# nevi-me/rust-dataframe

Hardware: AMD Instinct MI355X
Metric: rows/sec filter+sum over 1e9 f64 Arrow rows; %HBM bw at 1/2/4/8 GPU (higher is better)
Workload: dtype f64

## Files before the change

rust_dataframe_amd/csrc/rdf_capi.cpp:

```cpp
#include <hip/hip_runtime.h>

#include <algorithm>
#include <cmath>
#include <cstdarg>
#include <cstdio>
#include <chrono>
#include <functional>
#include <cstring>
#include <map>
#include <memory>
#include <mutex>
#include <condition_variable>
#include <string>
#include <thread>
#include <vector>
#include <sys/syscall.h>
#include <unistd.h>

#include "rdf_device.h"
#include "rdf_stage_copy.h"
#include "rdf_utf8.h"

using namespace rdfk;

// ... 3 lines not shown
struct Arena {
    char*  base = nullptr;
    size_t cap = 0, used = 0, wanted = 0;
    std::vector<void*> overflow;
};

struct Ctx {
    bool        ready = false;
    int         device = 0;
    hipStream_t own_stream = nullptr;
    hipStream_t stream = nullptr;
    hipStream_t copy_stream = nullptr;
    bool copy_pending = false;
    Arena       arena;
    char*       pinned = nullptr;
    size_t      pinned_cap = 0;
    std::string err;
    std::string last_kernel;
    bool   opt_spec = true;
    bool   opt_fast_filter = true;
    bool   opt_vec_bitmap = false;
    bool   opt_filter_one = true;
    int    opt_filter_gen = 2;
    int    opt_filter_block = 1;
    int    opt_interp_lean = 1;
    int    opt_filter_owned = 1;
    int    opt_filter_ends = 1;
    int    opt_filter_mixed = 0;
    int    opt_filter_short = 1;
    int    opt_filter_block_rows = 8192;
// ... 9 lines not shown
    int    opt_sort_msd = 1;
    int    opt_sort_sample = 1;
    int    opt_join_table = 2;
    int    opt_jit = 1;
    int    opt_take_rows = 1;
    int    opt_gb_skew_plan = 1;
    int    opt_gb_compact = 1;
    int64_t opt_comm_max_bytes = 0;
    int    opt_spec_blocks = 0;
    int    opt_spec_tile_rot = -1;
    int    opt_spec_xcd_swz = -1;
    int    opt_spec_grid_adj = 0;
    int    opt_gspec_blocks = 0;
    int    opt_gb_hot = 1;
    int    opt_gb_bucket = 0;
    int    opt_gb_partition = 3;
    bool   timing = false;
    std::vector<std::pair<hipEvent_t, hipEvent_t>> events;
    size_t events_used = 0;
    std::multimap<size_t, void*> pool_free;
    size_t pool_cached = 0;
    int64_t opt_stream_slab = 0;
    void*  sbuf_dev[2] = {nullptr, nullptr};
    void*  sbuf_pin[2] = {nullptr, nullptr};
    size_t sbuf_dev_cap = 0, sbuf_pin_cap = 0;
    hipEvent_t sbuf_ev[2] = {nullptr, nullptr};
    void*  dbuf_dev[2] = {nullptr, nullptr};
    void*  dbuf_pin[2] = {nullptr, nullptr};
    size_t dbuf_dev_cap = 0, dbuf_pin_cap = 0;
    hipEvent_t dbuf_ev[2] = {nullptr, nullptr};
// ... 5 lines not shown
    char* tab_pin = nullptr; size_t tab_pin_cap = 0, tab_pin_used = 0;
    bool   agg_comm_entered = false;
    ::rdf_comm* agg_comm = nullptr;
    ~Ctx();
};

thread_local Ctx g_ctx;

Ctx::~Ctx() {
    if (!ready || (long)syscall(SYS_gettid) == (long)getpid()) return;
    (void)hipSetDevice(device);
    if (stream) (void)hipStreamSynchronize(stream);
    for (void* p : arena.overflow) (void)hipFree(p);
    if (arena.base) (void)hipFree(arena.base);
    if (pinned) (void)hipHostFree(pinned);
    for (auto& kv : pool_free) (void)hipFree(kv.second);
    for (int b = 0; b < 2; ++b) { if (sbuf_dev[b]) (void)hipFree(sbuf_dev[b]); if (sbuf_pin[b]) (void)hipHostFree(sbuf_pin[b]); if (sbuf_ev[b]) (void)hipEventDestroy(sbuf_ev[b]); }
    if (tab_pin) (void)hipHostFree(tab_pin);
    if (d2h_stream) (void)hipStreamSynchronize(d2h_stream);
    for (int b = 0; b < 2; ++b) { if (dbuf_dev[b]) (void)hipFree(dbuf_dev[b]); if (dbuf_pin[b]) (void)hipHostFree(dbuf_pin[b]); if (dbuf_ev[b]) (void)hipEventDestroy(dbuf_ev[b]); }
    if (d2h_stream) (void)hipStreamDestroy(d2h_stream);
    for (auto& ev : events) { (void)hipEventDestroy(ev.first); (void)hipEventDestroy(ev.second); }
    if (copy_stream) { (void)hipStreamSynchronize(copy_stream); (void)hipStreamDestroy(copy_stream); }
    if (own_stream) (void)hipStreamDestroy(own_stream);
    ready = false;
}

rdf_status fail(rdf_status st, const char* fmt, ...) {
    char buf[512];
    va_list ap;
// ... 24 lines not shown
    if (e != hipSuccess || n <= 0)
        return fail(RDF_DEVICE_ERROR, "no HIP device visible (%s); librdf_mi355x has no CPU fallback",
                    e != hipSuccess ? hipGetErrorString(e) : "device count 0");
    HIP_TRY(hipGetDevice(&c.device));
    hipDeviceProp_t prop;
    HIP_TRY(hipGetDeviceProperties(&prop, c.device));
    if (strncmp(prop.gcnArchName, "gfx950", 6) != 0)
        return fail(RDF_DEVICE_ERROR, "device %d is %s; this library carries gfx950 (MI355X) code only", c.device, prop.gcnArchName);
    HIP_TRY(hipStreamCreateWithFlags(&c.own_stream, hipStreamNonBlocking));
    c.stream = c.own_stream;
    if (const char* e = getenv("RDF_SPEC_BLOCKS_PER_CU")) { const int v = atoi(e); if (v >= 0 && v <= 8) c.opt_spec_blocks = v; }
    if (const char* e = getenv("RDF_SPEC_TILE_ROT")) c.opt_spec_tile_rot = atoi(e);
    if (const char* e = getenv("RDF_SPEC_XCD_SWZ")) c.opt_spec_xcd_swz = atoi(e);
    if (const char* e = getenv("RDF_SPEC_GRID_ADJ")) c.opt_spec_grid_adj = atoi(e);
    if (const char* e = getenv("RDF_STREAM_TABLE_KERNEL")) c.opt_stream_table_kernel = atoi(e) != 0;
    if (const char* e = getenv("RDF_GSPEC_BLOCKS_PER_CU")) { const int v = atoi(e); if (v >= 0 && v <= 8) c.opt_gspec_blocks = v; }
    c.ready = true;
    return RDF_OK;
}

void arena_begin() {
    Arena& a = g_ctx.arena;
    for (void* p : a.overflow) (void)hipFree(p);
    a.overflow.clear();
    if (a.wanted > a.cap) {
        if (a.base) (void)hipFree(a.base);
        a.base = nullptr;
        a.cap = 0;
        size_t want = a.wanted + a.wanted / 4 + (1u << 20);
        void* p = nullptr;
// ... 11 lines not shown
        a.used += bytes;
        return RDF_OK;
    }
    void* p = nullptr;
    hipError_t e = hipMalloc(&p, bytes);
    if (e != hipSuccess) return fail(RDF_MEMORY_ERROR, "hipMalloc(%zu) failed: %s", bytes, hipGetErrorString(e));
    a.overflow.push_back(p);
    *out = p;
    return RDF_OK;
}
rdf_status pinned_reserve(size_t bytes) {
    Ctx& c = g_ctx;
    if (bytes <= c.pinned_cap) return RDF_OK;
    if (c.pinned && c.stream) (void)hipStreamSynchronize(c.stream);
    if (c.pinned) (void)hipHostFree(c.pinned);
    c.pinned = nullptr;
    c.pinned_cap = 0;
    size_t want = bytes + bytes / 2 + 4096;
    void* p = nullptr;
    hipError_t e = hipHostMalloc(&p, want, hipHostMallocDefault);
    if (e != hipSuccess) return fail(RDF_MEMORY_ERROR, "hipHostMalloc(%zu) failed: %s", want, hipGetErrorString(e));
    c.pinned = (char*)p;
    c.pinned_cap = want;
    return RDF_OK;
}

constexpr size_t kPoolGranule = (size_t)2 << 20;
constexpr size_t kPoolMaxCached = (size_t)96 << 30;
rdf_status pool_alloc(size_t bytes, void** out, size_t* got) {
    Ctx& c = g_ctx;
    const size_t gran = bytes < ((size_t)1 << 20) ? (size_t)4096 : kPoolGranule;
    const size_t want = (bytes + 256 + gran - 1) / gran * gran;
    auto it = c.pool_free.lower_bound(want);
    if (it != c.pool_free.end() && it->first <= want + want / 4 + gran) {
        *out = it->second; *got = it->first;
        c.pool_cached -= it->first;
        c.pool_free.erase(it);
        return RDF_OK;
// ... 749 lines not shown
                    if (op == RDF_OP_ADD) h = LH_I_ADD;
                    else if (op == RDF_OP_MUL) h = LH_I_MUL;
                    else if (op == RDF_OP_SUB) h = sw ? LH_I_RSUB : LH_I_SUB;
                }
            } break;
            default: break;
        }
        if (h == LH_NONE) return false;
        lean.code[i].swapped = (uint8_t)((in.swapped & 1) | (h << 1));
    }
    return true;
}

rdf_status launch_agg_pair(const EvalArgs* ea, const FilterAggF64Args* fa, int cmp, int feat, int grid, int nvalues,
                           const int* cls, AggPartial* partials, AggPartial* result, const char* spec_sig = nullptr,
                           const SpecArgs* sa = nullptr) {
    Ctx& c = g_ctx;
    KernelTimer kt;
    if (sa) {
        const bool jit = jit_find(spec_sig) != nullptr;
        c.last_kernel = std::string("spec_kernel<") + spec_sig + ">" + (jit ? " [compiled at run time]" : "");
        const hipError_t le = launch_spec(spec_sig, *sa, grid, c.stream);
        if (le != hipSuccess && jit) { (void)hipGetLastError(); return kRetryInterpreted; }
        if (le != hipSuccess) return fail(RDF_DEVICE_ERROR, "launch_spec: %s", hipGetErrorString(le));
    }
    else if (fa) { c.last_kernel = "filter_agg_f64_kernel"; HIP_TRY(launch_filter_agg_f64(*fa, cmp, grid, c.stream)); }
    else {
        EvalArgs lean;
        if (c.opt_interp_lean && feat == 0 && lean_assign(*ea, lean)) { c.last_kernel = "eval_kernel<AGG, lean>"; HIP_TRY(launch_eval_lean(lean, SINK_AGG, grid, c.stream, c.opt_interp_lean == 2)); }
        else { c.last_kernel = "eval_kernel<AGG>"; HIP_TRY(launch_eval(*ea, SINK_AGG, feat, grid, c.stream)); }
    }
    kt.stop();
    AggFinalArgs f;
    memset(&f, 0, sizeof f);
    f.partials = partials;
    f.result = result;
    f.nblocks = grid;
    f.nvalues = nvalues;
    for (int k = 0; k < nvalues; ++k) f.value_cls[k] = cls[k];
    HIP_TRY(launch_agg_final(f, c.stream));
    return RDF_OK;
}

void fill_agg_result(rdf_agg_result* r, int dt, const AggPartial& p) {
    memset(r, 0, sizeof *r);
    r->dtype = dt;
    r->count = p.cnt;
// ... 309 lines not shown
        tile_start.assign((size_t)nchunks + 1, 0);
        for (int64_t c = 0; c < nchunks; ++c) tile_start[(size_t)c + 1] = tile_start[(size_t)c] + (clen[(size_t)c] + kEvalTile - 1) / kEvalTile;
    }
    const int64_t ntiles = fc ? eval_tiles->ntiles : tile_start[(size_t)nchunks];
    int grid = (int)(ntiles < (int64_t)eval_grid_limit() ? ntiles : (int64_t)eval_grid_limit());

    const size_t n_nc = ps.sink == RDF_SINK_STORE ? (size_t)ps.nvalues * (size_t)nchunks : 0;
    const int gwords = grouped ? group_words(ps.ngroups, ps.nvalues) : 0;
    const size_t scratch_bytes = 16 + n_nc * 8 + ((size_t)grid + 4) * (grouped ? (size_t)gwords * 8 : (size_t)ps.nvalues * sizeof(AggPartial));
    void* scratch = nullptr;
    RDF_TRY(arena_alloc(scratch_bytes, &scratch));
    uint32_t* d_flags = (uint32_t*)scratch;
    int64_t* d_nullc = (int64_t*)((char*)scratch + 16);
    AggPartial* d_partials = (AggPartial*)((char*)scratch + 16 + n_nc * 8);
    AggPartial* d_result = d_partials + (size_t)grid * (size_t)ps.nvalues;
    HIP_TRY(hipMemsetAsync(scratch, 0, 16 + n_nc * 8, ctx.stream));

    EvalArgs ea;
    memset(&ea, 0, sizeof ea);
    ea.nchunks = nchunks;
    ea.ntiles = ntiles;
    ea.ncols = ncols;
    ea.nvalues = ps.nvalues;
    ea.ncode = (int)cc.code.size();
    ea.ntmp = cc.tmp_max;
    ea.flags = d_flags;
    ea.out_null_counts = d_nullc;
    ea.partials = d_partials;
    for (int k = 0; k < ncols; ++k) ea.col_dtype[k] = col_dtype[k];
    int cls[kMaxGroupValues] = {0, 0, 0, 0, 0, 0, 0, 0};
    for (int v = 0; v < ps.nvalues; ++v) { cls[v] = value_class(value_dtype[v]); ea.value_cls[v] = cls[v]; }
// ... 277 lines not shown
                    const DevChunkCol& y = in_dev[(size_t)vr.column];
                    const uintptr_t xa = (uintptr_t)((const double*)x.values + x.offset), ya = (uintptr_t)((const double*)y.values + y.offset);
                    if ((xa & 7) == 0 && (ya & 7) == 0 && (xa & 15) == (ya & 15)) {
                        memset(&fa, 0, sizeof fa);
                        fa.x = (const double*)x.values; fa.x_validity = x.validity; fa.x_offset = x.offset;
                        fa.y = (const double*)y.values; fa.y_validity = y.validity; fa.y_offset = y.offset;
                        fa.n = clen[0];
                        const uint64_t cu = cc.imm_for(*sc, RDF_F64);
                        memcpy(&fa.c, &cu, 8);
                        fa.partials = d_partials;
                        fast = true;
                    }
                }
            }
        }
        if (use_spec) {
            const rdf_status ls = launch_agg_pair(nullptr, nullptr, 0, 0, grid, ps.nvalues, cls, d_partials, d_result, sp.sig.c_str(), &sa);
            if (ls == kRetryInterpreted) return run_program(ps, cols, ncols, nchunks, outs, aggs, len_mismatch_msg, fc);
            RDF_TRY(ls);
        } else if (fast) {
            const int64_t per_block = (int64_t)kBlock * 4 * 2;
            int64_t want = (clen[0] + per_block - 1) / per_block;
            grid = (int)(want < (int64_t)eval_grid_limit() ? want : (int64_t)eval_grid_limit());
            if (grid < 1) grid = 1;
            d_result = d_partials + (size_t)grid * (size_t)ps.nvalues;
            RDF_TRY(launch_agg_pair(nullptr, &fa, cmp, 0, grid, 1, cls, d_partials, d_result));
        } else {
            RDF_TRY(launch_agg_pair(&ea, nullptr, 0, cc.feat(), grid, ps.nvalues, cls, d_partials, d_result));
        }
        if (ctx.agg_comm) {
            AggPartial hp[kMaxValues];
            uint32_t flags = 0;
            RDF_TRY(agg_dist_finish(*ctx.agg_comm, d_result, d_flags, ps.nvalues, cls, hp, &flags));
            if (flags & 2u) return fail(RDF_COMPUTE_ERROR, "pipeline_dist: another rank failed before the combine");
            if (flags & 1u) return fail(RDF_DIVIDE_BY_ZERO, "Divide by zero error");
            for (int v = 0; v < ps.nvalues; ++v) fill_agg_result(&aggs[v], value_dtype[v], hp[v]);
            return RDF_OK;
        }
        RDF_TRY(pinned_reserve(pin_off + 64 + sizeof(AggPartial) * kMaxValues));
        char* pin = ctx.pinned + pin_off;
        HIP_TRY(hipMemcpyAsync(pin, d_flags, 16, hipMemcpyDeviceToHost, ctx.stream));
        HIP_TRY(hipMemcpyAsync(pin + 64, d_result, sizeof(AggPartial) * (size_t)ps.nvalues, hipMemcpyDeviceToHost, ctx.stream));
        HIP_TRY(hipStreamSynchronize(ctx.stream));
        dbg.mark("kernel + result");
        uint32_t flags;
        memcpy(&flags, pin, 4);
        if (flags & 1u) return fail(RDF_DIVIDE_BY_ZERO, "Divide by zero error");
        for (int v = 0; v < ps.nvalues; ++v) {
            AggPartial p;
            memcpy(&p, pin + 64 + sizeof(AggPartial) * (size_t)v, sizeof p);
            fill_agg_result(&aggs[v], value_dtype[v], p);
        }
        return RDF_OK;
    }

    {
        KernelTimer kt;
// ... 125 lines not shown

rdf_status rdf_set_device(int32_t device) {
    Ctx& c = g_ctx;
    if (c.ready && c.device == device) return RDF_OK;
    if (c.ready) {
        (void)hipStreamSynchronize(c.stream);
        for (void* p : c.arena.overflow) (void)hipFree(p);
        c.arena.overflow.clear();
        if (c.arena.base) (void)hipFree(c.arena.base);
        c.arena = Arena();
        for (auto& ev : c.events) { (void)hipEventDestroy(ev.first); (void)hipEventDestroy(ev.second); }
        c.events.clear();
        c.events_used = 0;
        if (c.own_stream) (void)hipStreamDestroy(c.own_stream);
        c.own_stream = c.stream = nullptr;
        c.ready = false;
    }
    HIP_TRY(hipSetDevice(device));
    return ensure_ready();
}

rdf_status rdf_set_stream(void* hip_stream) {
    RDF_TRY(ensure_ready());
    g_ctx.stream = hip_stream ? (hipStream_t)hip_stream : g_ctx.own_stream;
    return RDF_OK;
}

rdf_status rdf_synchronize(void) {
    RDF_TRY(ensure_ready());
    HIP_TRY(hipStreamSynchronize(g_ctx.stream));
// ... 2414 lines not shown
    else if (strcmp(name, "gspec_blocks_per_cu") == 0) g_ctx.opt_gspec_blocks = (int)value;
    else if (strcmp(name, "filter_gen") == 0) g_ctx.opt_filter_gen = (int)value;
    else if (strcmp(name, "filter_fused") == 0) g_ctx.opt_filter_fused = (int)value;
    else if (strcmp(name, "filter_block") == 0) g_ctx.opt_filter_block = value == 3 ? 3 : value != 0;
    else if (strcmp(name, "interp_lean") == 0) g_ctx.opt_interp_lean = value == 2 ? 2 : value != 0;
    else if (strcmp(name, "sort_super") == 0) {
        if (value > 100) g_ctx.opt_sort_super_force = value > 164 ? 64 : (int)value - 100;
        else { g_ctx.opt_sort_super_force = 0; g_ctx.opt_sort_super = value < 1 ? 1 : value > 64 ? 64 : (int)value; }
    }
    else if (strcmp(name, "filter_owned") == 0) g_ctx.opt_filter_owned = value == 2 ? 2 : value != 0;
    else if (strcmp(name, "filter_ends") == 0) g_ctx.opt_filter_ends = value != 0;
    else if (strcmp(name, "filter_mixed") == 0) g_ctx.opt_filter_mixed = value == 2 ? 2 : value != 0;
    else if (strcmp(name, "filter_short") == 0) g_ctx.opt_filter_short = value != 0;
    else if (strcmp(name, "filter_block_rows") == 0) g_ctx.opt_filter_block_rows = value < 1 ? 1 : (int)value;
    else if (strcmp(name, "filter_lookback") == 0) g_ctx.opt_filter_lookback = value == 1 ? 1 : value == 2 ? 2 : 3;
    else if (strcmp(name, "comm_max_bytes") == 0) g_ctx.opt_comm_max_bytes = value;
    else if (strcmp(name, "stream_slab_bytes") == 0) g_ctx.opt_stream_slab = value;
    else return fail(RDF_INVALID_ARGUMENT, "unknown option %s", name);
    return RDF_OK;
}
int32_t rdf_spec_catalog_size(void) { return spec_catalog_size(); }
const char* rdf_jit_status(void) {
    thread_local std::string line;
    line = jit_status();
    return line.c_str();
}
const char* rdf_last_kernel(void) { return g_ctx.last_kernel.c_str(); }

rdf_status rdf_probe_stream(int32_t kind, const void* a, void* b, void* c, int64_t bytes, int32_t reps, double* best_gbps, char* shape, int32_t shape_len) {
    if (kind < 0 || kind > 2 || !a || (kind >= 1 && !b) || (kind == 2 && !c) || bytes < 16 || !best_gbps) return fail(RDF_INVALID_ARGUMENT, "probe_stream: kind 0..2 with its device buffers, bytes >= 16");
// ... 65 lines not shown
```

rust_dataframe_amd/csrc/rdf_common.hip.h:

```cpp
#pragma once
#include "rdf_device.h"

namespace rdfk {

__device__ __forceinline__ uint64_t uniform64(uint64_t v) {
    uint32_t lo = __builtin_amdgcn_readfirstlane((uint32_t)v);
    uint32_t hi = __builtin_amdgcn_readfirstlane((uint32_t)(v >> 32));
    return ((uint64_t)hi << 32) | lo;
}
__device__ __forceinline__ int wave_id() { return __builtin_amdgcn_readfirstlane((int)(threadIdx.x >> 6)); }

template <class T> using GlobalPtr = const T __attribute__((address_space(1)))*;
template <class T> using GlobalMutPtr = T __attribute__((address_space(1)))*;
template <class T> __device__ __forceinline__ GlobalPtr<T> as_global(const void* p) { return (GlobalPtr<T>)p; }
template <class T> using ConstPtr = const T __attribute__((address_space(4)))*;
template <class T> __device__ __forceinline__ ConstPtr<T> as_const(const void* p) { return (ConstPtr<T>)p; }
__device__ __forceinline__ DevChunkCol const_col(const DevChunkCol* table, int64_t i) {
    const ConstPtr<DevChunkCol> t = as_const<DevChunkCol>(table);
    DevChunkCol c;
    c.values = t[i].values; c.validity = t[i].validity; c.offset = t[i].offset;
    return c;
}
template <class T> __device__ __forceinline__ GlobalMutPtr<T> as_global_mut(void* p) { return (GlobalMutPtr<T>)p; }

// ... 116 lines not shown
    if (cls == CLS_F64) {
        sum = d2u(u2d(sum) + u2d(s2));
        mn = d2u(fmin(u2d(mn), u2d(mn2)));
        mx = d2u(fmax(u2d(mx), u2d(mx2)));
    } else if (cls == CLS_SIGNED) {
        sum += s2;
        mn = (uint64_t)((int64_t)mn2 < (int64_t)mn ? (int64_t)mn2 : (int64_t)mn);
        mx = (uint64_t)((int64_t)mx2 > (int64_t)mx ? (int64_t)mx2 : (int64_t)mx);
    } else {
        sum += s2;
        mn = mn2 < mn ? mn2 : mn;
        mx = mx2 > mx ? mx2 : mx;
    }
}

__device__ __forceinline__ void block_reduce_agg(int cls, uint64_t sum, uint64_t mn, uint64_t mx, int64_t cnt,
                                                 AggPartial* lds4, AggPartial* out) {
#pragma unroll
    for (int m = 32; m >= 1; m >>= 1) {
        uint64_t s2 = shfl_xor64(sum, m), mn2 = shfl_xor64(mn, m), mx2 = shfl_xor64(mx, m);
        int64_t c2 = (int64_t)shfl_xor64((uint64_t)cnt, m);
        agg_merge(cls, sum, mn, mx, cnt, s2, mn2, mx2, c2);
    }
    const int wave = threadIdx.x >> 6;
    __syncthreads();
    if ((threadIdx.x & 63) == 0) { lds4[wave].sum = sum; lds4[wave].mn = mn; lds4[wave].mx = mx; lds4[wave].cnt = cnt; }
    __syncthreads();
    if (threadIdx.x == 0) {
        uint64_t s = lds4[0].sum, a = lds4[0].mn, b = lds4[0].mx;
        int64_t c = lds4[0].cnt;
        for (int w = 1; w < kBlock / 64; ++w) agg_merge(cls, s, a, b, c, lds4[w].sum, lds4[w].mn, lds4[w].mx, lds4[w].cnt);
        out->sum = s; out->mn = a; out->mx = b; out->cnt = c;
    }
}

__device__ __forceinline__ void trig_reduce(double x, double& r, int& q) {
    const double kd = rint(x * 6.36619772367581382433e-01);
    q = (int)kd;
    double t = fma(-kd, 1.57079632673412561417e+00, x);
    t = fma(-kd, 6.07710050630396597660e-11, t);
    t = fma(-kd, 2.02226624871116645580e-21, t);
    r = fma(-kd, 8.47842766036889956997e-32, t);
}
__device__ __forceinline__ double trig_ksin(double r) {
    const double z = r * r, v = z * r;
    const double p = fma(z, fma(z, fma(z, fma(z, 1.58969099521155010221e-10, -2.50507602534068634195e-08), 2.75573137070700676789e-06),
                                -1.98412698298579493134e-04), 8.33333333332248946124e-03);
// ... 222 lines not shown
```

rust_dataframe_amd/csrc/rdf_device.h:

```cpp
#pragma once
#include "rdf_sort_map.h"
#include <stdint.h>
#include <hip/hip_runtime.h>

#include <string>
#include "../../include/rdf_mi355x.h"

namespace rdfk {

constexpr int kBlock = 256;
constexpr int kVPT = 4;
constexpr int kEvalTile = kBlock * kVPT;
constexpr int kFilterTile = 4096;
constexpr int kFilterTileSmall = 1024;
constexpr int kMaxCode = 56;
constexpr int kMaxCols = 8;
constexpr int kMaxFrameCols = 64;
constexpr int kPreCols = 4;
constexpr int kMaxTmp = 4;
constexpr int kMaxValues = RDF_MAX_VALUES;
constexpr int kMaxGroupValues = RDF_MAX_GROUP_VALUES;
constexpr int kMaxFilterCols = 8;

struct DevChunkCol {
// ... 19 lines not shown
    uint16_t src;
    uint64_t imm;
};
static_assert(sizeof(Instr) == 16, "Instr must stay 16 bytes");
enum : int {
    LH_NONE = 0, LH_LOAD, LH_STORE_TMP, LH_FILTER, LH_EMIT, LH_NOT, LH_CAST_I2F, LH_CAST_U2F,
    LH_F_GT, LH_F_GE, LH_F_EQ, LH_F_NE, LH_F_LT, LH_F_LE, LH_F_ADD, LH_F_SUB, LH_F_RSUB, LH_F_MUL, LH_F_DIV, LH_F_RDIV,
    LH_I_ADD, LH_I_SUB, LH_I_RSUB, LH_I_MUL, LH_AND, LH_OR
};

struct AggPartial {
    uint64_t sum, mn, mx;
    int64_t  cnt;
};
enum : int32_t { CLS_F64 = 0, CLS_SIGNED = 1, CLS_UNSIGNED = 2 };

enum : int32_t { SINK_STORE = 0, SINK_AGG = 1, SINK_GROUP = 2 };

struct EvalArgs {
    const DevChunkCol* cols;
    const int64_t*     chunk_tile_start;
    const int64_t*     chunk_len;
    DevOutChunk*       outs;
    int64_t*           out_null_counts;
    AggPartial*        partials;
    uint64_t*          group_partials;
    uint32_t*          flags;
    int64_t            nchunks, ntiles;
    DevChunkCol        inline_cols[kMaxCols];
    DevOutChunk        inline_outs[kMaxValues];
    int64_t            inline_len;
    int32_t            ncols, nvalues, ncode, ntmp;
    int32_t            col_dtype[kMaxCols];
    int32_t            value_cls[kMaxGroupValues];
    int32_t            ngroups, group_replicas;
    Instr              code[kMaxCode];
};

inline __host__ __device__ int group_words(int ngroups, int nvalues) { return (ngroups + 1) * (2 * nvalues + 1); }

constexpr int kGSpecCols = 8;
constexpr int kGSpecImm = 8;
struct GSpecArgs {
    const DevChunkCol* cols_tab;
    const int64_t*     chunk_tile_start;
    const int64_t*     chunk_len;
    DevChunkCol        cols[kGSpecCols];
    int32_t            col_map[kGSpecCols];
    int64_t            nchunks, ntiles, n;
    uint64_t           imm[kGSpecImm];
// ... 11 lines not shown
};

struct AggFinalArgs {
    const AggPartial* partials;
    AggPartial*       result;
    int32_t           nblocks, nvalues;
    int32_t           value_cls[kMaxValues];
};

struct FilterAggF64Args {
    const double*  x;   const uint8_t* x_validity;   int64_t x_offset;
    const double*  y;   const uint8_t* y_validity;   int64_t y_offset;
    int64_t        n;
    double         c;
    AggPartial*    partials;
};

constexpr int kSpecCols = 8;
constexpr int kSpecImm = 8;
struct SpecArgs {
    DevChunkCol        cols[kSpecCols];
    DevOutChunk        out;
    const DevChunkCol* cols_tab;
    const DevOutChunk* outs_tab;
    const int64_t*     chunk_tile_start;
    const int64_t*     chunk_len;
    int64_t            nchunks, ntiles;
    int64_t            n;
    uint64_t           tile_inv;
    uint64_t           imm[kSpecImm];
    int64_t*           out_null_count;
    AggPartial*        partials;
    uint32_t*          flags;
    int32_t            vec_bitmap;
    int32_t            rt[8];
    int32_t            alias[kSpecCols];
    int64_t            tile_rot;
    int32_t            xcd_swz, pad0;
};

struct MaskTables {
    const DevChunkCol* mask;
    const int64_t*     chunk_tile_start;
    const int64_t*     chunk_len;
    int64_t            nchunks, ntiles;
};
struct FilterArgs {
    MaskTables         t;
    const DevChunkCol* cols;
    DevOutChunk*       outs;
    int64_t*           out_null_counts;
    const int64_t*     tile_scan;
    int32_t            ncols;
// ... 545 lines not shown
```

rust_dataframe_amd/csrc/rdf_eval.hip:

```cpp
#include "rdf_common.hip.h"

#ifndef RDF_FEAT
#error "compile with -DRDF_FEAT=0|1|2"
#endif

namespace rdfk {


__device__ __forceinline__ uint64_t cast_value(int from, int to, uint64_t x, bool& ok) {
    ok = true;
    if (from == to) return x;
    double f = 0.0;
    bool src_float = false;
    if (from == RDF_F64) { f = u2d(x); src_float = true; }
    else if (from == RDF_F32) { f = (double)u2f(x); src_float = true; }
    if (to == RDF_BOOL) return src_float ? (uint64_t)(f != 0.0) : (uint64_t)(x != 0);
    if (to == RDF_F64) {
        if (src_float) return d2u(f);
        return d2u(dt_is_signed(from) ? (double)(int64_t)x : (double)x);
    }
    if (to == RDF_F32) {
        if (from == RDF_F64) return f2u((float)u2d(x));
        return f2u(dt_is_signed(from) ? (float)(int64_t)x : (float)x);
    }
// ... 666 lines not shown
            const bool fsum = w < a.nvalues * gS && a.value_cls[(w / gS) & (kMaxGroupValues - 1)] == CLS_F64;
            uint64_t acc0 = gtab[w];
            for (int r = 1; r < a.group_replicas; ++r) {
                const uint64_t x = gtab[(size_t)r * gwords + w];
                acc0 = fsum ? d2u(u2d(acc0) + u2d(x)) : acc0 + x;
            }
            a.group_partials[(size_t)blockIdx.x * gwords + w] = acc0;
        }
    }
    if (SINK == SINK_AGG) {
#pragma unroll
        for (int k = 0; k < NVAL; ++k)
            if (k < a.nvalues)
                block_reduce_agg(a.value_cls[k], g_sum[k], g_mn[k], g_mx[k], g_cnt[k], red_lds,
                                 &a.partials[(int64_t)blockIdx.x * a.nvalues + k]);
    }
}


template <int SINK, int NPRE, int NVAL>
static void launch_one(const EvalArgs& a, int grid, size_t lds, hipStream_t s) {
    hipLaunchKernelGGL((eval_kernel<RDF_FEAT, SINK, NPRE, NVAL>), dim3(grid), dim3(kBlock), lds, s, a);
}
template <int SINK>
static void launch_shape(const EvalArgs& a, int npre, int nval, int grid, size_t lds, hipStream_t s) {
    if (nval <= 1) {
        if (npre <= 1) launch_one<SINK, 1, 1>(a, grid, lds, s);
        else if (npre <= 2) launch_one<SINK, 2, 1>(a, grid, lds, s);
        else launch_one<SINK, 4, 1>(a, grid, lds, s);
    } else if (nval <= 2) {
// ... 22 lines not shown
```

rust_dataframe_amd/csrc/rdf_eval_lean.hip:

```cpp
#include "rdf_common.hip.h"

namespace rdfk {

#define RDF_ROWS _Pragma("unroll") for (int j = 0; j < kVPT; ++j)

typedef uint64_t lean_u64x2 __attribute__((ext_vector_type(2)));
typedef uint32_t lean_u32x2 __attribute__((ext_vector_type(2)));

__device__ __forceinline__ uint32_t lean_nibble(const uint64_t (&w)[kVPT], int lane) {
    const uint32_t q = (uint32_t)lane >> 4, sh = ((uint32_t)lane & 15u) * 4u;
    const uint32_t c0 = (uint32_t)(w[0] >> sh), c1 = (uint32_t)(w[1] >> sh), c2 = (uint32_t)(w[2] >> sh), c3 = (uint32_t)(w[3] >> sh);
    const uint32_t m0 = 0u - (uint32_t)(q == 0), m1 = 0u - (uint32_t)(q == 1), m2 = 0u - (uint32_t)(q == 2), m3 = 0u - (uint32_t)(q == 3);
    return ((c0 & m0) | (c1 & m1) | (c2 & m2) | (c3 & m3)) & 15u;
}

__device__ __forceinline__ void lean_load8(const DevChunkCol cc, int64_t rw, int64_t clen, bool full, uint64_t (&v)[kVPT], uint32_t& valid) {
    const int lane = threadIdx.x & 63;
    const GlobalPtr<uint64_t> base = as_global<uint64_t>(cc.values) + cc.offset;
    if (full && (((uintptr_t)cc.values + (uintptr_t)(cc.offset + rw) * 8) & 15) == 0) {
        const GlobalPtr<lean_u64x2> p = (GlobalPtr<lean_u64x2>)(base + rw + (int64_t)lane * kVPT);
        const lean_u64x2 a0 = __builtin_nontemporal_load(p), a1 = __builtin_nontemporal_load(p + 1);
        v[0] = a0[0]; v[1] = a0[1]; v[2] = a1[0]; v[3] = a1[1];
    } else {
        const int64_t last = clen - 1;
// ... 54 lines not shown
__device__ __forceinline__ void lean_block_reduce(int cls, uint64_t sum, uint64_t mn, uint64_t mx, int64_t cnt, AggPartial* lds4, AggPartial* out) {
#pragma unroll
    for (int m = 32; m >= 1; m >>= 1) {
        const uint64_t s2 = shfl_xor64(sum, m), mn2 = shfl_xor64(mn, m), mx2 = shfl_xor64(mx, m);
        const int64_t c2 = (int64_t)shfl_xor64((uint64_t)cnt, m);
        agg_merge(cls, sum, mn, mx, cnt, s2, mn2, mx2, c2);
    }
    sum = uniform64(sum); mn = uniform64(mn); mx = uniform64(mx); cnt = (int64_t)uniform64((uint64_t)cnt);
    const int wave = wave_id();
    __syncthreads();
    lds4[wave].sum = sum; lds4[wave].mn = mn; lds4[wave].mx = mx; lds4[wave].cnt = cnt;
    __syncthreads();
    uint64_t s = lds4[0].sum, lo = lds4[0].mn, hi = lds4[0].mx;
    int64_t c = lds4[0].cnt;
    for (int w = 1; w < kBlock / 64; ++w) agg_merge(cls, s, lo, hi, c, lds4[w].sum, lds4[w].mn, lds4[w].mx, lds4[w].cnt);
    out->sum = s; out->mn = lo; out->mx = hi; out->cnt = c;
}

__device__ __forceinline__ void lean_store_words(uint8_t* bitmap, int64_t rw, int64_t rows_left, uint32_t nibble, int lane) {
    uint64_t x = (uint64_t)(nibble & 15u) << (((uint32_t)lane & 15u) * 4u);
#pragma unroll
    for (int m = 1; m < 16; m <<= 1) x |= shfl_xor64(x, m);
    const int64_t span = rows_left < 0 ? 0 : rows_left < (int64_t)kVPT * 64 ? rows_left : (int64_t)kVPT * 64;
    const int nwords = (int)((span + 63) >> 6);
    const __amdgpu_buffer_rsrc_t rs = __builtin_amdgcn_make_buffer_rsrc(bitmap + (rw >> 6) * 8, 0, nwords * 8, 0x00020000);
    lean_u32x2 w;
    w[0] = (uint32_t)x; w[1] = (uint32_t)(x >> 32);
    const uint32_t off = ((uint32_t)lane & 15u) == 0 ? ((uint32_t)lane >> 4) * 8u : 0x7FFFFFF0u;
    __builtin_amdgcn_raw_buffer_store_b64(w, rs, (int)off, 0, 0);
}

// ... 238 lines not shown
                        } else {
                            const uint64_t* tv = tmp_vals + (size_t)src * R * kBlock + tid;
                            RDF_ROWS_R opnd[r] = tv[r * kBlock];
                            opv = tmp_valid[src * kBlock + tid];
                        }
                        accv &= opv;
                        lean_bin<R>(h, acc, [&](int r) { return opnd[r]; }, accv & inr, err);
                    }
                } break;
            }
        }
        tile = ntile;
        have = nhave;
    }

    if (__ballot(err != 0) != 0) *(volatile uint32_t*)a.flags = 1u;
    if constexpr (SINK == SINK_AGG) {
#pragma unroll
        for (int k = 0; k < NVAL; ++k)
            if (k < a.nvalues)
                lean_block_reduce(a.value_cls[k], g_sum[k], g_mn[k], g_mx[k], g_cnt[k], red_lds, &a.partials[(int64_t)blockIdx.x * a.nvalues + k]);
    }
}

template <int SINK, int NPRE, int NVAL, int T>
static void lean_launch_one(const EvalArgs& a, int grid, hipStream_t s) {
    const size_t lds = (size_t)a.ntmp * ((size_t)T * kVPT * kBlock * 8 + kBlock * 4);
    hipLaunchKernelGGL((eval_lean_kernel<SINK, NPRE, NVAL, T>), dim3(grid), dim3(kBlock), lds, s, a);
}

hipError_t launch_eval_lean(const EvalArgs& a, int sink, int grid, hipStream_t s, bool one_tile) {
    const int npre = a.ncols, nval = a.nvalues;
    const bool two = !one_tile && (npre <= 1 || (npre <= 2 && sink == SINK_AGG)) && (size_t)a.ntmp * (2 * kVPT * kBlock * 8 + kBlock * 4) <= 65536;
    if (sink == SINK_STORE) {
        if (npre <= 1) { if (two) lean_launch_one<SINK_STORE, 1, 1, 2>(a, grid, s); else lean_launch_one<SINK_STORE, 1, 1, 1>(a, grid, s); }
        else if (npre <= 2) lean_launch_one<SINK_STORE, 2, 1, 1>(a, grid, s);
// ... 14 lines not shown
```

rust_dataframe_amd/csrc/rdf_kernels.hip:

```cpp
#include "rdf_common.hip.h"
#include "rdf_join_place.h"

namespace rdfk {

__global__ __launch_bounds__(kBlock) void agg_final_kernel(const AggFinalArgs a) {
    __shared__ AggPartial red_lds[kBlock / 64];
    for (int k = 0; k < a.nvalues; ++k) {
        const int cls = a.value_cls[k];
        uint64_t s, mn, mx;
        int64_t cnt;
        agg_init(cls, s, mn, mx, cnt);
        for (int b = threadIdx.x; b < a.nblocks; b += kBlock) {
            const AggPartial p = a.partials[(int64_t)b * a.nvalues + k];
            agg_merge(cls, s, mn, mx, cnt, p.sum, p.mn, p.mx, p.cnt);
        }
        block_reduce_agg(cls, s, mn, mx, cnt, red_lds, &a.result[k]);
        __syncthreads();
    }
}


template <int CMP>
__device__ __forceinline__ bool cmp_f64(double x, double c) {
    if (CMP == RDF_OP_GT) return x > c;
    if (CMP == RDF_OP_GE) return x >= c;
    if (CMP == RDF_OP_EQ) return x == c;
    if (CMP == RDF_OP_NE) return x != c;
    if (CMP == RDF_OP_LT) return x < c;
    return x <= c;
}

struct F64Agg {
    double sum, mn, mx;
// ... 58 lines not shown
#pragma unroll
        for (int u = 0; u < kFU; ++u) {
            const int64_t i = wbase + u * 64 + lane;
            uint32_t bits = i < nvec ? 3u : 0u;
            if (HASV) {
                const int sh = (2 * lane) & 63;
                if (a.x_validity) bits &= (uint32_t)((lane < 32 ? wx[2 * u] : wx[2 * u + 1]) >> sh) & 3u;
                if (!SAME && a.y_validity) bits &= (uint32_t)((lane < 32 ? wy[2 * u] : wy[2 * u + 1]) >> sh) & 3u;
            }
            const dvec2 yy = SAME ? vx[u] : vy[u];
            if ((bits & 1u) && cmp_f64<CMP>(vx[u].x, a.c)) g.add(yy.x);
            if ((bits & 2u) && cmp_f64<CMP>(vx[u].y, a.c)) g.add(yy.y);
        }
    }
    block_reduce_agg(CLS_F64, d2u(g.sum), d2u(g.mn), d2u(g.mx), g.cnt, red_lds, &a.partials[blockIdx.x]);
}

template <int WW> constexpr int filter_tile_rows() { return WW * 64 * (kBlock / 64); }
static_assert(filter_tile_rows<16>() == kFilterTile && filter_tile_rows<4>() == kFilterTileSmall, "tile sizes of the two instantiations");

template <int WW>
__device__ __forceinline__ void locate_tile(const MaskTables& t, int64_t tile, int64_t& c, int64_t& r0, int64_t& clen) {
    c = t.nchunks == 1 ? 0 : find_chunk_tile(t.chunk_tile_start, t.nchunks, tile);
    r0 = (tile - t.chunk_tile_start[c]) * filter_tile_rows<WW>();
    clen = t.chunk_len[c];
}

template <int kWW>
__device__ __forceinline__ void keep_words(const DevChunkCol& m, int64_t rw, int64_t clen, uint64_t (&kw)[kWW]) {
    load_windows<kWW>((const uint8_t*)m.values, m.offset + rw, clen - rw, kw);
// ... 1760 lines not shown
```

rust_dataframe_amd/csrc/rdf_spec_kernel.hip.h:

```cpp
#pragma once
#include <map>
#include <string>
#include <type_traits>

#include "rdf_expr.hip.h"

namespace rdfk {


template <int DT> struct AggT;
template <> struct AggT<RDF_F64> {
    double sum, mn, mx; int64_t cnt;
    static constexpr int cls = CLS_F64;
    __device__ __forceinline__ void init() { sum = 0.0; mn = mx = __longlong_as_double(0x7FF8000000000000ll); cnt = 0; }
    __device__ __forceinline__ void add(double v) { sum += v; mn = fmin(mn, v); mx = fmax(mx, v); ++cnt; }
    __device__ __forceinline__ uint64_t s() const { return d2u(sum); }
    __device__ __forceinline__ uint64_t a() const { return d2u(mn); }
    __device__ __forceinline__ uint64_t b() const { return d2u(mx); }
};
template <> struct AggT<RDF_I64> {
    uint64_t sum; int64_t mn, mx; int64_t cnt;
    static constexpr int cls = CLS_SIGNED;
    __device__ __forceinline__ void init() { sum = 0; mn = INT64_MAX; mx = INT64_MIN; cnt = 0; }
    __device__ __forceinline__ void add(int64_t v) { sum += (uint64_t)v; mn = v < mn ? v : mn; mx = v > mx ? v : mx; ++cnt; }
// ... 405 lines not shown
                }
#pragma unroll
                for (int e = 0; e < RV; ++e) nulls += (uint32_t)__popcll(inb[e] & ~vb[e]);
            }
            if (lane < R && rw + 64 * lane < n) {
                if constexpr (V0::dt == RDF_BOOL) as_global_mut<uint64_t>(out.values)[(rw >> 6) + lane] = word_val;
                if (out.validity) as_global_mut<uint64_t>(out.validity)[(rw >> 6) + lane] = word_vld;
            }
        }
    }
    if (c.err) atomicOr(a.flags, c.err);
    if constexpr (P::SINK == SINK_AGG) {
        constexpr int nv = has_v1 ? 2 : 1;
        block_reduce_agg(g0.cls, g0.s(), g0.a(), g0.b(), g0.cnt, red_lds, &a.partials[(int64_t)blockIdx.x * nv]);
        if constexpr (has_v1) block_reduce_agg(g1.cls, g1.s(), g1.a(), g1.b(), g1.cnt, red_lds, &a.partials[(int64_t)blockIdx.x * nv + 1]);
    } else {
        if (cur_chunk >= 0 && lane == 0 && nulls) atomicAdd((unsigned long long*)&a.out_null_count[cur_chunk], (unsigned long long)nulls);
    }
}


typedef void (*SpecLaunch)(const SpecArgs&, int, hipStream_t);
struct SpecEntry { SpecLaunch launch; int rows_per_tile; };
std::map<std::string, SpecEntry>& spec_registry();

template <class P>
static void launch_prog(const SpecArgs& a, int grid, hipStream_t s) {
    hipLaunchKernelGGL((spec_kernel<P>), dim3(grid), dim3(kBlock), 0, s, a);
}
template <class P>
// ... 119 lines not shown
```

Baseline: 841.6 billion.

## Fold final aggregate into main kernel via last-block ticket and host-mapped output

Measured after the change: 841.8 billion, median of 6. Within noise of the previous version (+0.0%).

```diff
diff --git a/rust_dataframe_amd/csrc/rdf_capi.cpp b/rust_dataframe_amd/csrc/rdf_capi.cpp
--- a/rust_dataframe_amd/csrc/rdf_capi.cpp
+++ b/rust_dataframe_amd/csrc/rdf_capi.cpp
@@ -41,6 +41,7 @@
     bool copy_pending = false;
     Arena       arena;
     char*       pinned = nullptr;
+    char*       pinned_dev = nullptr;
     size_t      pinned_cap = 0;
     std::string err;
     std::string last_kernel;
@@ -80,6 +81,9 @@
     int    opt_gspec_blocks = 0;
     int    opt_gb_hot = 1;
     int    opt_gb_bucket = 0;
+    int    opt_agg_fold = 1;
+    void*  fold_state = nullptr;
+    uint64_t fold_t0 = 0;
     int    opt_gb_partition = 3;
     bool   timing = false;
     std::vector<std::pair<hipEvent_t, hipEvent_t>> events;
@@ -115,6 +119,7 @@
     for (void* p : arena.overflow) (void)hipFree(p);
     if (arena.base) (void)hipFree(arena.base);
     if (pinned) (void)hipHostFree(pinned);
+    if (fold_state) (void)hipFree(fold_state);
     for (auto& kv : pool_free) (void)hipFree(kv.second);
     for (int b = 0; b < 2; ++b) { if (sbuf_dev[b]) (void)hipFree(sbuf_dev[b]); if (sbuf_pin[b]) (void)hipHostFree(sbuf_pin[b]); if (sbuf_ev[b]) (void)hipEventDestroy(sbuf_ev[b]); }
     if (tab_pin) (void)hipHostFree(tab_pin);
@@ -169,6 +174,7 @@
     if (const char* e = getenv("RDF_SPEC_XCD_SWZ")) c.opt_spec_xcd_swz = atoi(e);
     if (const char* e = getenv("RDF_SPEC_GRID_ADJ")) c.opt_spec_grid_adj = atoi(e);
     if (const char* e = getenv("RDF_STREAM_TABLE_KERNEL")) c.opt_stream_table_kernel = atoi(e) != 0;
+    if (const char* e = getenv("RDF_AGG_FOLD")) c.opt_agg_fold = atoi(e) != 0;
     if (const char* e = getenv("RDF_GSPEC_BLOCKS_PER_CU")) { const int v = atoi(e); if (v >= 0 && v <= 8) c.opt_gspec_blocks = v; }
     c.ready = true;
     return RDF_OK;
@@ -210,14 +216,35 @@
     if (bytes <= c.pinned_cap) return RDF_OK;
     if (c.pinned && c.stream) (void)hipStreamSynchronize(c.stream);
     if (c.pinned) (void)hipHostFree(c.pinned);
-    c.pinned = nullptr;
+    c.pinned = c.pinned_dev = nullptr;
     c.pinned_cap = 0;
     size_t want = bytes + bytes / 2 + 4096;
     void* p = nullptr;
     hipError_t e = hipHostMalloc(&p, want, hipHostMallocDefault);
     if (e != hipSuccess) return fail(RDF_MEMORY_ERROR, "hipHostMalloc(%zu) failed: %s", want, hipGetErrorString(e));
+    void* pd = nullptr;
+    e = hipHostGetDevicePointer(&pd, p, 0);
+    if (e != hipSuccess) { (void)hipHostFree(p); return fail(RDF_MEMORY_ERROR, "hipHostGetDevicePointer: %s", hipGetErrorString(e)); }
     c.pinned = (char*)p;
+    c.pinned_dev = (char*)pd;
     c.pinned_cap = want;
+    return RDF_OK;
+}
+
+rdf_status agg_fold_state(AggFold* fold) {
+    Ctx& c = g_ctx;
+    if (!c.fold_state) {
+        void* p = nullptr;
+        HIP_TRY(hipMalloc(&p, 256));
+        const hipError_t e = hipMemsetAsync(p, 0, 256, c.stream) == hipSuccess ? hipStreamSynchronize(c.stream) : hipGetLastError();
+        if (e != hipSuccess) { (void)hipFree(p); return fail(RDF_DEVICE_ERROR, "agg_fold state: %s", hipGetErrorString(e)); }
+        c.fold_state = p;
+        c.fold_t0 = 0;
+    }
+    memset(fold, 0, sizeof *fold);
+    fold->ticket = (unsigned long long*)c.fold_state;
+    fold->flags = (uint32_t*)((char*)c.fold_state + 64);
+    fold->t0 = c.fold_t0;
     return RDF_OK;
 }
 
@@ -997,23 +1024,36 @@
 
 rdf_status launch_agg_pair(const EvalArgs* ea, const FilterAggF64Args* fa, int cmp, int feat, int grid, int nvalues,
                            const int* cls, AggPartial* partials, AggPartial* result, const char* spec_sig = nullptr,
-                           const SpecArgs* sa = nullptr) {
+                           const SpecArgs* sa = nullptr, const AggFold* fold = nullptr) {
     Ctx& c = g_ctx;
     KernelTimer kt;
     if (sa) {
         const bool jit = jit_find(spec_sig) != nullptr;
         c.last_kernel = std::string("spec_kernel<") + spec_sig + ">" + (jit ? " [compiled at run time]" : "");
-        const hipError_t le = launch_spec(spec_sig, *sa, grid, c.stream);
+        SpecArgs a = *sa;
+        if (fold) a.fold = *fold;
+        const hipError_t le = launch_spec(spec_sig, a, grid, c.stream);
         if (le != hipSuccess && jit) { (void)hipGetLastError(); return kRetryInterpreted; }
         if (le != hipSuccess) return fail(RDF_DEVICE_ERROR, "launch_spec: %s", hipGetErrorString(le));
     }
-    else if (fa) { c.last_kernel = "filter_agg_f64_kernel"; HIP_TRY(launch_filter_agg_f64(*fa, cmp, grid, c.stream)); }
+    else if (fa) {
+        c.last_kernel = "filter_agg_f64_kernel";
+        FilterAggF64Args a = *fa;
+        if (fold) a.fold = *fold;
+        HIP_TRY(launch_filter_agg_f64(a, cmp, grid, c.stream));
+    }
     else {
         EvalArgs lean;
-        if (c.opt_interp_lean && feat == 0 && lean_assign(*ea, lean)) { c.last_kernel = "eval_kernel<AGG, lean>"; HIP_TRY(launch_eval_lean(lean, SINK_AGG, grid, c.stream, c.opt_interp_lean == 2)); }
-        else { c.last_kernel = "eval_kernel<AGG>"; HIP_TRY(launch_eval(*ea, SINK_AGG, feat, grid, c.stream)); }
+        EvalArgs a = *ea;
+        if (fold) a.fold = *fold;
+        if (c.opt_interp_lean && feat == 0 && lean_assign(a, lean)) { c.last_kernel = "eval_kernel<AGG, lean>"; HIP_TRY(launch_eval_lean(lean, SINK_AGG, grid, c.stream, c.opt_interp_lean == 2)); }
+        else { c.last_kernel = "eval_kernel<AGG>"; HIP_TRY(launch_eval(a, SINK_AGG, feat, grid, c.stream)); }
     }
     kt.stop();
+    if (fold) {
+        c.fold_t0 += (uint64_t)grid;
+        return RDF_OK;
+    }
     AggFinalArgs f;
     memset(&f, 0, sizeof f);
     f.partials = partials;
@@ -1353,7 +1393,8 @@
     int64_t* d_nullc = (int64_t*)((char*)scratch + 16);
     AggPartial* d_partials = (AggPartial*)((char*)scratch + 16 + n_nc * 8);
     AggPartial* d_result = d_partials + (size_t)grid * (size_t)ps.nvalues;
-    HIP_TRY(hipMemsetAsync(scratch, 0, 16 + n_nc * 8, ctx.stream));
+    const bool agg_fold = ps.sink == RDF_SINK_AGG && !grouped && ctx.opt_agg_fold;
+    if (!agg_fold) HIP_TRY(hipMemsetAsync(scratch, 0, 16 + n_nc * 8, ctx.stream));
 
     EvalArgs ea;
     memset(&ea, 0, sizeof ea);
@@ -1661,8 +1702,20 @@
                 }
             }
         }
+        AggFold fold;
+        if (agg_fold) {
+            RDF_TRY(pinned_reserve(pin_off + 64 + sizeof(AggPartial) * kMaxValues));
+            RDF_TRY(agg_fold_state(&fold));
+            fold.result = d_result;
+            fold.call_flags = d_flags;
+            fold.host = ctx.pinned_dev + pin_off;
+            fold.nvalues = ps.nvalues;
+            for (int v = 0; v < ps.nvalues; ++v) fold.value_cls[v] = cls[v];
+            ea.flags = sa.flags = fold.flags;
+        }
+        const AggFold* fp = agg_fold ? &fold : nullptr;
         if (use_spec) {
-            const rdf_status ls = launch_agg_pair(nullptr, nullptr, 0, 0, grid, ps.nvalues, cls, d_partials, d_result, sp.sig.c_str(), &sa);
+            const rdf_status ls = launch_agg_pair(nullptr, nullptr, 0, 0, grid, ps.nvalues, cls, d_partials, d_result, sp.sig.c_str(), &sa, fp);
             if (ls == kRetryInterpreted) return run_program(ps, cols, ncols, nchunks, outs, aggs, len_mismatch_msg, fc);
             RDF_TRY(ls);
         } else if (fast) {
@@ -1671,9 +1724,10 @@
             grid = (int)(want < (int64_t)eval_grid_limit() ? want : (int64_t)eval_grid_limit());
             if (grid < 1) grid = 1;
             d_result = d_partials + (size_t)grid * (size_t)ps.nvalues;
-            RDF_TRY(launch_agg_pair(nullptr, &fa, cmp, 0, grid, 1, cls, d_partials, d_result));
+            if (agg_fold) fold.result = d_result;
+            RDF_TRY(launch_agg_pair(nullptr, &fa, cmp, 0, grid, 1, cls, d_partials, d_result, nullptr, nullptr, fp));
         } else {
-            RDF_TRY(launch_agg_pair(&ea, nullptr, 0, cc.feat(), grid, ps.nvalues, cls, d_partials, d_result));
+            RDF_TRY(launch_agg_pair(&ea, nullptr, 0, cc.feat(), grid, ps.nvalues, cls, d_partials, d_result, nullptr, nullptr, fp));
         }
         if (ctx.agg_comm) {
             AggPartial hp[kMaxValues];
@@ -1686,8 +1740,10 @@
         }
         RDF_TRY(pinned_reserve(pin_off + 64 + sizeof(AggPartial) * kMaxValues));
         char* pin = ctx.pinned + pin_off;
-        HIP_TRY(hipMemcpyAsync(pin, d_flags, 16, hipMemcpyDeviceToHost, ctx.stream));
-        HIP_TRY(hipMemcpyAsync(pin + 64, d_result, sizeof(AggPartial) * (size_t)ps.nvalues, hipMemcpyDeviceToHost, ctx.stream));
+        if (!agg_fold) {
+            HIP_TRY(hipMemcpyAsync(pin, d_flags, 16, hipMemcpyDeviceToHost, ctx.stream));
+            HIP_TRY(hipMemcpyAsync(pin + 64, d_result, sizeof(AggPartial) * (size_t)ps.nvalues, hipMemcpyDeviceToHost, ctx.stream));
+        }
         HIP_TRY(hipStreamSynchronize(ctx.stream));
         dbg.mark("kernel + result");
         uint32_t flags;
@@ -1843,6 +1899,9 @@
         c.events_used = 0;
         if (c.own_stream) (void)hipStreamDestroy(c.own_stream);
         c.own_stream = c.stream = nullptr;
+        if (c.fold_state) (void)hipFree(c.fold_state);
+        c.fold_state = nullptr;
+        c.fold_t0 = 0;
         c.ready = false;
     }
     HIP_TRY(hipSetDevice(device));
@@ -4287,6 +4346,7 @@
     else if (strcmp(name, "filter_short") == 0) g_ctx.opt_filter_short = value != 0;
     else if (strcmp(name, "filter_block_rows") == 0) g_ctx.opt_filter_block_rows = value < 1 ? 1 : (int)value;
     else if (strcmp(name, "filter_lookback") == 0) g_ctx.opt_filter_lookback = value == 1 ? 1 : value == 2 ? 2 : 3;
+    else if (strcmp(name, "agg_fold") == 0) g_ctx.opt_agg_fold = value != 0;
     else if (strcmp(name, "comm_max_bytes") == 0) g_ctx.opt_comm_max_bytes = value;
     else if (strcmp(name, "stream_slab_bytes") == 0) g_ctx.opt_stream_slab = value;
     else return fail(RDF_INVALID_ARGUMENT, "unknown option %s", name);
diff --git a/rust_dataframe_amd/csrc/rdf_common.hip.h b/rust_dataframe_amd/csrc/rdf_common.hip.h
--- a/rust_dataframe_amd/csrc/rdf_common.hip.h
+++ b/rust_dataframe_amd/csrc/rdf_common.hip.h
@@ -154,6 +154,13 @@
     }
 }
 
+__device__ __forceinline__ void agg_store_partial(AggPartial* out, uint64_t s, uint64_t mn, uint64_t mx, int64_t c) {
+    __hip_atomic_store(&out->sum, s, __ATOMIC_RELAXED, __HIP_MEMORY_SCOPE_AGENT);
+    __hip_atomic_store(&out->mn, mn, __ATOMIC_RELAXED, __HIP_MEMORY_SCOPE_AGENT);
+    __hip_atomic_store(&out->mx, mx, __ATOMIC_RELAXED, __HIP_MEMORY_SCOPE_AGENT);
+    __hip_atomic_store(&out->cnt, c, __ATOMIC_RELAXED, __HIP_MEMORY_SCOPE_AGENT);
+}
+
 __device__ __forceinline__ void block_reduce_agg(int cls, uint64_t sum, uint64_t mn, uint64_t mx, int64_t cnt,
                                                  AggPartial* lds4, AggPartial* out) {
 #pragma unroll
@@ -170,7 +177,46 @@
         uint64_t s = lds4[0].sum, a = lds4[0].mn, b = lds4[0].mx;
         int64_t c = lds4[0].cnt;
         for (int w = 1; w < kBlock / 64; ++w) agg_merge(cls, s, a, b, c, lds4[w].sum, lds4[w].mn, lds4[w].mx, lds4[w].cnt);
-        out->sum = s; out->mn = a; out->mx = b; out->cnt = c;
+        agg_store_partial(out, s, a, b, c);
+    }
+}
+
+__device__ __forceinline__ void agg_fold_block(const AggPartial* partials, int nblocks, int nvalues, const int32_t (&value_cls)[kMaxValues],
+                                               AggPartial* lds4, AggPartial* result) {
+    for (int k = 0; k < nvalues; ++k) {
+        const int cls = value_cls[k];
+        uint64_t s, mn, mx;
+        int64_t cnt;
+        agg_init(cls, s, mn, mx, cnt);
+        for (int b = threadIdx.x; b < nblocks; b += kBlock) {
+            const AggPartial p = partials[(int64_t)b * nvalues + k];
+            agg_merge(cls, s, mn, mx, cnt, p.sum, p.mn, p.mx, p.cnt);
+        }
+        block_reduce_agg(cls, s, mn, mx, cnt, lds4, &result[k]);
+        __syncthreads();
+    }
+}
+
+__device__ __forceinline__ void agg_fold_finish(const AggFold& f, const AggPartial* partials, AggPartial* lds4) {
+    asm volatile("s_waitcnt vmcnt(0)" ::: "memory");
+    __syncthreads();
+    if (threadIdx.x == 0) {
+        const unsigned long long t = __hip_atomic_fetch_add(f.ticket, 1ull, __ATOMIC_RELAXED, __HIP_MEMORY_SCOPE_AGENT);
+        const bool last = t == f.t0 + gridDim.x - 1;
+        if (last) {
+            __builtin_amdgcn_fence(__ATOMIC_ACQUIRE, "agent");
+            asm volatile("s_waitcnt vmcnt(0)" ::: "memory");
+        }
+        lds4[0].cnt = last ? 1 : 0;
+    }
+    __syncthreads();
+    if (lds4[0].cnt == 0) return;
+    agg_fold_block(partials, gridDim.x, f.nvalues, f.value_cls, lds4, f.result);
+    if (threadIdx.x == 0) {
+        const uint32_t fl = __hip_atomic_exchange(f.flags, 0u, __ATOMIC_RELAXED, __HIP_MEMORY_SCOPE_AGENT);
+        for (int k = 0; k < f.nvalues; ++k) ((AggPartial*)(f.host + 64))[k] = f.result[k];
+        *(uint32_t*)f.host = fl;
+        f.call_flags[0] = fl; f.call_flags[1] = 0; f.call_flags[2] = 0; f.call_flags[3] = 0;
     }
 }
 
diff --git a/rust_dataframe_amd/csrc/rdf_device.h b/rust_dataframe_amd/csrc/rdf_device.h
--- a/rust_dataframe_amd/csrc/rdf_device.h
+++ b/rust_dataframe_amd/csrc/rdf_device.h
@@ -57,6 +57,17 @@
     int64_t  cnt;
 };
 enum : int32_t { CLS_F64 = 0, CLS_SIGNED = 1, CLS_UNSIGNED = 2 };
+
+struct AggFold {
+    unsigned long long* ticket;
+    uint32_t*    flags;
+    AggPartial*  result;
+    uint32_t*    call_flags;
+    char*        host;
+    uint64_t     t0;
+    int32_t      nvalues, pad;
+    int32_t      value_cls[kMaxValues];
+};
 
 enum : int32_t { SINK_STORE = 0, SINK_AGG = 1, SINK_GROUP = 2 };
 
@@ -77,6 +88,7 @@
     int32_t            col_dtype[kMaxCols];
     int32_t            value_cls[kMaxGroupValues];
     int32_t            ngroups, group_replicas;
+    AggFold            fold;
     Instr              code[kMaxCode];
 };
 
@@ -118,6 +130,7 @@
     int64_t        n;
     double         c;
     AggPartial*    partials;
+    AggFold        fold;
 };
 
 constexpr int kSpecCols = 8;
@@ -141,6 +154,7 @@
     int32_t            alias[kSpecCols];
     int64_t            tile_rot;
     int32_t            xcd_swz, pad0;
+    AggFold            fold;
 };
 
 struct MaskTables {
diff --git a/rust_dataframe_amd/csrc/rdf_eval.hip b/rust_dataframe_amd/csrc/rdf_eval.hip
--- a/rust_dataframe_amd/csrc/rdf_eval.hip
+++ b/rust_dataframe_amd/csrc/rdf_eval.hip
@@ -704,6 +704,7 @@
             if (k < a.nvalues)
                 block_reduce_agg(a.value_cls[k], g_sum[k], g_mn[k], g_mx[k], g_cnt[k], red_lds,
                                  &a.partials[(int64_t)blockIdx.x * a.nvalues + k]);
+        if (a.fold.ticket) agg_fold_finish(a.fold, a.partials, red_lds);
     }
 }
 
diff --git a/rust_dataframe_amd/csrc/rdf_eval_lean.hip b/rust_dataframe_amd/csrc/rdf_eval_lean.hip
--- a/rust_dataframe_amd/csrc/rdf_eval_lean.hip
+++ b/rust_dataframe_amd/csrc/rdf_eval_lean.hip
@@ -92,7 +92,60 @@
     uint64_t s = lds4[0].sum, lo = lds4[0].mn, hi = lds4[0].mx;
     int64_t c = lds4[0].cnt;
     for (int w = 1; w < kBlock / 64; ++w) agg_merge(cls, s, lo, hi, c, lds4[w].sum, lds4[w].mn, lds4[w].mx, lds4[w].cnt);
-    out->sum = s; out->mn = lo; out->mx = hi; out->cnt = c;
+    agg_store_partial(out, s, lo, hi, c);
+}
+
+__device__ __forceinline__ uint64_t lean_lane0_ticket(unsigned long long* p) {
+    uint64_t old = 0, save;
+    asm volatile("s_mov_b64 %1, exec\n\ts_mov_b64 exec, 1\n\tglobal_atomic_add_x2 %0, %2, %3, off sc0\n\ts_waitcnt vmcnt(0)\n\ts_mov_b64 exec, %1"
+                 : "+v"(old), "=&s"(save) : "v"(p), "v"((uint64_t)1) : "memory");
+    return uniform64(old);
+}
+__device__ __forceinline__ void lean_lane0_or(uint32_t* p, uint32_t bits) {
+    uint64_t save;
+    asm volatile("s_mov_b64 %0, exec\n\ts_mov_b64 exec, 1\n\tglobal_atomic_or %1, %2, off\n\ts_mov_b64 exec, %0"
+                 : "=&s"(save) : "v"(p), "v"(bits) : "memory");
+}
+
+__device__ __forceinline__ void lean_fold_finish(const AggFold& f, const AggPartial* partials, AggPartial* lds4) {
+    asm volatile("s_waitcnt vmcnt(0)" ::: "memory");
+    __syncthreads();
+    if (wave_id() == 0) {
+        const uint64_t t = lean_lane0_ticket(f.ticket);
+        const bool last = t == f.t0 + gridDim.x - 1;
+        if (last) {
+            __builtin_amdgcn_fence(__ATOMIC_ACQUIRE, "agent");
+            asm volatile("s_waitcnt vmcnt(0)" ::: "memory");
+        }
+        lds4[0].cnt = last ? 1 : 0;
+    }
+    __syncthreads();
+    if (uniform64((uint64_t)lds4[0].cnt) == 0) return;
+    const int nblocks = (int)gridDim.x;
+    for (int k = 0; k < f.nvalues; ++k) {
+        const int cls = f.value_cls[k];
+        uint64_t s, mn, mx;
+        int64_t cnt;
+        agg_init(cls, s, mn, mx, cnt);
+        for (int b0 = 0; b0 < nblocks; b0 += kBlock) {
+            const int b = b0 + (int)threadIdx.x;
+            const AggPartial p = partials[(int64_t)(b < nblocks ? b : nblocks - 1) * f.nvalues + k];
+            uint64_t s2 = s, mn2 = mn, mx2 = mx;
+            int64_t c2 = cnt;
+            agg_merge(cls, s2, mn2, mx2, c2, p.sum, p.mn, p.mx, p.cnt);
+            const bool in = b < nblocks;
+            s = in ? s2 : s; mn = in ? mn2 : mn; mx = in ? mx2 : mx; cnt = in ? c2 : cnt;
+        }
+        lean_block_reduce(cls, s, mn, mx, cnt, lds4, &f.result[k]);
+        __syncthreads();
+    }
+    if (wave_id() == 0) {
+        const uint32_t fl = __builtin_amdgcn_readfirstlane(__hip_atomic_load(f.flags, __ATOMIC_RELAXED, __HIP_MEMORY_SCOPE_AGENT));
+        __hip_atomic_store(f.flags, 0u, __ATOMIC_RELAXED, __HIP_MEMORY_SCOPE_AGENT);
+        for (int k = 0; k < f.nvalues; ++k) ((AggPartial*)(f.host + 64))[k] = f.result[k];
+        *(uint32_t*)f.host = fl;
+        f.call_flags[0] = fl; f.call_flags[1] = 0; f.call_flags[2] = 0; f.call_flags[3] = 0;
+    }
 }
 
 __device__ __forceinline__ void lean_store_words(uint8_t* bitmap, int64_t rw, int64_t rows_left, uint32_t nibble, int lane) {
@@ -361,12 +414,13 @@
         have = nhave;
     }
 
-    if (__ballot(err != 0) != 0) *(volatile uint32_t*)a.flags = 1u;
+    if (__ballot(err != 0) != 0) lean_lane0_or(a.flags, 1u);
     if constexpr (SINK == SINK_AGG) {
 #pragma unroll
         for (int k = 0; k < NVAL; ++k)
             if (k < a.nvalues)
                 lean_block_reduce(a.value_cls[k], g_sum[k], g_mn[k], g_mx[k], g_cnt[k], red_lds, &a.partials[(int64_t)blockIdx.x * a.nvalues + k]);
+        if (a.fold.ticket) lean_fold_finish(a.fold, a.partials, red_lds);
     }
 }
 
diff --git a/rust_dataframe_amd/csrc/rdf_kernels.hip b/rust_dataframe_amd/csrc/rdf_kernels.hip
--- a/rust_dataframe_amd/csrc/rdf_kernels.hip
+++ b/rust_dataframe_amd/csrc/rdf_kernels.hip
@@ -5,18 +5,7 @@
 
 __global__ __launch_bounds__(kBlock) void agg_final_kernel(const AggFinalArgs a) {
     __shared__ AggPartial red_lds[kBlock / 64];
-    for (int k = 0; k < a.nvalues; ++k) {
-        const int cls = a.value_cls[k];
-        uint64_t s, mn, mx;
-        int64_t cnt;
-        agg_init(cls, s, mn, mx, cnt);
-        for (int b = threadIdx.x; b < a.nblocks; b += kBlock) {
-            const AggPartial p = a.partials[(int64_t)b * a.nvalues + k];
-            agg_merge(cls, s, mn, mx, cnt, p.sum, p.mn, p.mx, p.cnt);
-        }
-        block_reduce_agg(cls, s, mn, mx, cnt, red_lds, &a.result[k]);
-        __syncthreads();
-    }
+    agg_fold_block(a.partials, a.nblocks, a.nvalues, a.value_cls, red_lds, a.result);
 }
 
 
@@ -105,6 +94,7 @@
         }
     }
     block_reduce_agg(CLS_F64, d2u(g.sum), d2u(g.mn), d2u(g.mx), g.cnt, red_lds, &a.partials[blockIdx.x]);
+    if (a.fold.ticket) agg_fold_finish(a.fold, a.partials, red_lds);
 }
 
 template <int WW> constexpr int filter_tile_rows() { return WW * 64 * (kBlock / 64); }
diff --git a/rust_dataframe_amd/csrc/rdf_spec_kernel.hip.h b/rust_dataframe_amd/csrc/rdf_spec_kernel.hip.h
--- a/rust_dataframe_amd/csrc/rdf_spec_kernel.hip.h
+++ b/rust_dataframe_amd/csrc/rdf_spec_kernel.hip.h
@@ -443,6 +443,7 @@
         constexpr int nv = has_v1 ? 2 : 1;
         block_reduce_agg(g0.cls, g0.s(), g0.a(), g0.b(), g0.cnt, red_lds, &a.partials[(int64_t)blockIdx.x * nv]);
         if constexpr (has_v1) block_reduce_agg(g1.cls, g1.s(), g1.a(), g1.b(), g1.cnt, red_lds, &a.partials[(int64_t)blockIdx.x * nv + 1]);
+        if (a.fold.ticket) agg_fold_finish(a.fold, a.partials, red_lds);
     } else {
         if (cur_chunk >= 0 && lane == 0 && nulls) atomicAdd((unsigned long long*)&a.out_null_count[cur_chunk], (unsigned long long)nulls);
     }
```
